# 0411tony/Yue

Measured on AMD Instinct MI355X. Metric: BPR triplet-updates/sec at k=128 (S-round semantics, user rows sequential; the reference's exact sequential semantics: secondary.exact), higher is better.
Workload: dtype f32

## Files before the change

yue_amd/csrc/bpr_host.hip:

```cpp
#include "host_common.hpp"

#include "train_kernels.hpp"
#include "round_kernels.hpp"

using yue_host::fail;
using yue_host::kr_of;
static_assert(yue::kNllSlots == yue_host::kNllSlotsHost && yue::kHeaderSlack == yue_host::kHeaderSlackHost, "host_common.hpp mirrors these");

namespace {

yue::TrainArgs make_args(yue_ctx *c, double lr, double regU, double regI) {
    yue::TrainArgs a{};
    a.P = c->P.p; a.Q = c->Q.p; a.dP = c->dP.p; a.dQ = c->dQ.p;
    a.stage = c->Q.p ? c->Q.p + (size_t)c->n * c->k : nullptr;
    a.ev_u = c->ev_u.p; a.ev_i = c->ev_i.p; a.ev_j = c->ev_j.p;
    a.indptr = c->indptr.p; a.indices = c->indices.p;
    a.nll_slots = c->scal.p;
    a.m = c->m; a.n = c->n; a.k = c->k;
    a.lr = lr;
    a.ru = (float)(lr * regU);
    a.ri = (float)(lr * regI);
    a.neg_lo = 0; a.neg_range = (int32_t)c->n;
    return a;
}
// ... 196 lines not shown
            default: return fail(YUE_ERR_ARG, "item matrices of 2 GiB and more: only the default events-per-wave setting (round_tpw = 0)");
        }
    } else
#define YUE_RM(KR_, TPW_) hipLaunchKernelGGL((yue::k_round_m<KR_, TPW_>), grid, block, 0, c->stream, a, ra, a.ev_u, a.ev_i, a.ev_j, mi, mj); break;
    switch (kr_of(c->k) * 16 + tpw) {
        case 1 * 16 + 8: YUE_RM(1, 8)
        case 1 * 16 + 16: YUE_RM(1, 16)
        case 2 * 16 + 8: YUE_RM(2, 8)
        case 4 * 16 + 4: YUE_RM(4, 4)
        case 1 * 16 + 4: YUE_RM(1, 4)
        case 2 * 16 + 4: YUE_RM(2, 4)
        case 1 * 16 + 2: YUE_RM(1, 2)
        case 2 * 16 + 2: YUE_RM(2, 2)
        default: return fail(YUE_ERR_ARG, "unsupported (k, TPW) combination");
    }
#undef YUE_RM
    launch_round_fold(c, a, e0, e1, round_index);
    return YUE_OK;
}

int launch_round_u(yue_ctx *c, const yue::TrainArgs &a, int64_t u0, int64_t u1, int64_t e0, int64_t e1, int64_t round_index) {
    yue::RoundUArgs ra{};
    ra.u_begin = u0; ra.u_end = u1; ra.ev_ptr = c->d_ev_ptr.p; ra.e_begin = e0; ra.e_end = e1; ra.staged = c->staged ? 1 : 0; ra.margins = c->margins.p;
    const int64_t blocks = (u1 - u0 + 3) / 4;
    if (blocks == 0) return YUE_OK;
    const dim3 grid((unsigned)blocks), block(256);
    const uint32_t *mi = c->meta_i.p, *mj = c->meta_j.p;
#define YUE_RU(KR_) do { if (c->opt_round_fast) hipLaunchKernelGGL((yue::k_round_u<KR_, true>), grid, block, 0, c->stream, a, ra, a.ev_i, a.ev_j, mi, mj); \
                         else hipLaunchKernelGGL((yue::k_round_u<KR_, false>), grid, block, 0, c->stream, a, ra, a.ev_i, a.ev_j, mi, mj); } while (0)
    switch (kr_of(c->k)) {
        case 1: YUE_RU(1); break;
        case 2: YUE_RU(2); break;
        default: YUE_RU(4); break;
    }
#undef YUE_RU
    launch_round_fold(c, a, e0, e1, round_index);
    return YUE_OK;
}

template <typename F>
int run_rounds(yue_ctx *c, yue::TrainArgs a, const std::vector<int64_t> &bounds, int apply_p, F after_round, bool meta = false, const std::vector<int64_t> *user_blocks = nullptr) {
    const int64_t R = (int64_t)bounds.size() - 1;
    int64_t widest = 0;
    for (int64_t r = 0; r < R; ++r) widest = std::max(widest, bounds[(size_t)r + 1] - bounds[(size_t)r]);
    if (widest >= (1ll << 24)) meta = false;
    const bool fits31 = (c->n + 2 * widest) * (int64_t)c->k * 4 < (1ll << 31);
// ... 73 lines not shown
}


}

namespace yue_host {
int zero_scalars(yue_ctx *c) {
    HIPCHK(hipMemsetAsync(c->scal.p, 0, (yue::kNllSlots + 8) * sizeof(double), c->stream));
    return YUE_OK;
}

int read_scalars(yue_ctx *c, double *nll, double *sp, double *sq) {
    double *sc = c->scal.p + yue::kNllSlots;
    hipLaunchKernelGGL(yue::k_sum_slots, dim3(1), dim3(64), 0, c->stream, c->scal.p, yue::kNllSlots, sc);
    double h[3];
    HIPCHK(hipMemcpyAsync(h, sc, sizeof h, hipMemcpyDeviceToHost, c->stream));
    HIPCHK(hipStreamSynchronize(c->stream));
    if (nll) *nll = h[0];
    if (sp) *sp = h[1];
    if (sq) *sq = h[2];
    return YUE_OK;
}

int sumsq_async(yue_ctx *c) {
    double *sc = c->scal.p + yue::kNllSlots;
    HIPCHK(hipMemsetAsync(sc + 1, 0, 2 * sizeof(double), c->stream));
    hipLaunchKernelGGL(yue::k_sumsq, dim3(2048), dim3(256), 0, c->stream, c->P.p, c->m * c->k, sc + 1);
    hipLaunchKernelGGL(yue::k_sumsq, dim3(2048), dim3(256), 0, c->stream, c->Q.p, c->n * c->k, sc + 2);
    return YUE_OK;
}

int upload_triplets(yue_ctx *c, const int32_t *u, const int32_t *i, const int32_t *j, int64_t T, bool validate) {
    for (int64_t t = 0; validate && t < T; ++t) {
        if (u[t] < 0 || u[t] >= c->m || i[t] < 0 || i[t] >= c->n || j[t] >= c->n)
            return fail(YUE_ERR_ARG, "triplet " + std::to_string(t) + " out of range");
    }
    HIPCHK(c->xu.resize((size_t)T + yue::kHeaderSlack)); HIPCHK(c->xi.resize((size_t)T + yue::kHeaderSlack)); HIPCHK(c->xj.resize((size_t)T + yue::kHeaderSlack));
    HIPCHK(hipMemcpyAsync(c->xu.p, u, T * sizeof(int32_t), hipMemcpyHostToDevice, c->stream));
    HIPCHK(hipMemcpyAsync(c->xi.p, i, T * sizeof(int32_t), hipMemcpyHostToDevice, c->stream));
    HIPCHK(hipMemcpyAsync(c->xj.p, j, T * sizeof(int32_t), hipMemcpyHostToDevice, c->stream));
    return YUE_OK;
}
}
using yue_host::zero_scalars; using yue_host::read_scalars; using yue_host::sumsq_async; using yue_host::upload_triplets;

extern "C" {

int yue_bpr_replay(yue_ctx *c, const int32_t *u, const int32_t *i, const int32_t *j, int64_t T,
                   double lr, double regU, double regI, double *nll_out) {
    if (!c || !c->have_factors) return fail(YUE_ERR_ARG, "yue_bpr_replay: no factors uploaded");
// ... 192 lines not shown
    double tot[2] = {(double)E, (double)c->n};
    if (yue_host::on_communicator(c)) {
        if ((rc = yue_allreduce_f64(c, tot, 2))) return rc;
        if ((rc = zero_scalars(c))) return rc;
    }
    const double etot = tot[0];
    if (round_events == 0 && (rc = default_round_events(c, tot[1] / c->nranks, &round_events))) return rc;
    int64_t ub = 1, group = 1;
    if ((rc = yue_epoch_plan(c->m, c->k, round_events, etot, c->nranks, &ub, &group, nullptr))) return rc;
    if (!yue_host::on_communicator(c)) group = std::max<int64_t>(1, (c->m + ub - 1) / ub);
    else group = std::max<int64_t>(1, ((int64_t)c->opt_comm_group_mb << 20) / std::max<int64_t>(1, ub * c->k * 4));
    std::vector<int64_t> ublock;
    for (int64_t u0 = 0; u0 < c->m; u0 += ub) { ublock.push_back(u0); bounds.push_back(c->h_ev_ptr[(size_t)u0]); }
    ublock.push_back(c->m); bounds.push_back(E);
    const int64_t R = (int64_t)ublock.size() - 1;
    const bool seq_user = !yue_host::on_communicator(c) && c->opt_round_user_seq && meta_path_fits(c);
    if (seq_user) {
        HIPCHK(c->d_ev_ptr.resize((size_t)c->m + 1));
        if (!c->d_ev_ptr_valid) {
            HIPCHK(hipMemcpyAsync(c->d_ev_ptr.p, c->h_ev_ptr.data(), ((size_t)c->m + 1) * sizeof(int64_t), hipMemcpyHostToDevice, c->stream));
            c->d_ev_ptr_valid = true;
        }
        HIPCHK(c->margins.resize((size_t)std::max<int64_t>(E, 1)));
    }
    c->last_round_user_seq = 0;
    auto after = [&](int64_t r) -> int {
        if (seq_user && !c->bigq) { c->last_round_user_seq = 1; return YUE_OK; }
        if ((r + 1) % group != 0 && r + 1 != R) return YUE_OK;
        const int64_t g_first = ublock[(size_t)(r - (r % group))], g_last = ublock[(size_t)r + 1];
        const int64_t first = g_first * c->k, count = (g_last - g_first) * c->k;
        const dim3 grid((unsigned)std::min<int64_t>(4096, (count + 255) / 256));
        if (!yue_host::on_communicator(c)) {
            hipLaunchKernelGGL(yue::k_apply_range, grid, dim3(256), 0, c->stream, c->P.p, c->dP.p, first, count);
            return YUE_OK;
        }
        HIPCHK(hipEventRecord(c->ev_rounds, c->stream));
        HIPCHK(hipStreamWaitEvent(c->comm_stream, c->ev_rounds, 0));
        c->comm_collectives += 1;
        c->comm_bytes += (double)count * sizeof(float);
        if (const int rcr = yue_host::reduce_user_block(c, first, count, c->comm_stream)) return rcr;
        hipLaunchKernelGGL(yue::k_apply_range, grid, dim3(256), 0, c->comm_stream, c->P.p, c->dP.p, first, count);
        return YUE_OK;
    };
    c->comm_collectives = 0; c->comm_bytes = 0.0; c->comm_wait_ms = 0.0;
    if ((rc = run_rounds(c, a, bounds, 0, after, meta_path_fits(c), seq_user ? &ublock : nullptr))) { reset_round_state(c); return rc; }
    if (c->last_round_user_seq && E > 0)
        hipLaunchKernelGGL(yue::k_loss_margins, dim3(2048), dim3(256), 0, c->stream, c->margins.p, c->ev_j.p, E, c->scal.p);
    if (yue_host::on_communicator(c)) {
        HIPCHK(hipEventRecord(c->ev_t_rounds, c->stream));
        HIPCHK(hipEventRecord(c->ev_t_comm, c->comm_stream));
    }
    HIPCHK(hipEventRecord(c->ev_comm, c->comm_stream));
    HIPCHK(hipStreamWaitEvent(c->stream, c->ev_comm, 0));
    c->comm_compute_waits = 1;
    HIPCHK(hipGetLastError());
    if ((rc = sumsq_async(c))) return rc;
    if ((rc = read_scalars(c, nll_out, sumsqP_out, sumsqQ_out))) return rc;
    if (yue_host::on_communicator(c)) {
        float ms = 0.f;
        HIPCHK(hipEventSynchronize(c->ev_t_comm));
        HIPCHK(hipEventElapsedTime(&ms, c->ev_t_rounds, c->ev_t_comm));
        c->comm_wait_ms = ms > 0.f ? ms : 0.0;
    }
    return YUE_OK;
}

int yue_epoch_plan(int64_t m, int k, int64_t round_events, double events_total, int nranks,
                   int64_t *user_block, int64_t *blocks_per_group, int64_t *n_blocks) {
    if (m <= 0 || k <= 0 || round_events <= 0 || nranks < 1 || !(events_total >= 0.0)) return fail(YUE_ERR_ARG, "yue_epoch_plan: bad argument");
    const double per_user = events_total / (double)nranks / (double)m;
    const int64_t ub = std::max<int64_t>(1, (int64_t)std::floor((double)round_events / std::max(per_user, 1e-9) + 0.5));
    if (user_block) *user_block = ub;
    if (blocks_per_group) *blocks_per_group = std::max<int64_t>(1, (8ll << 20) / std::max<int64_t>(1, ub * k * 4));
    if (n_blocks) *n_blocks = (m + ub - 1) / ub;
    return YUE_OK;
}

int yue_default_round_events(yue_ctx *c, int64_t *out) {
    if (!c || !c->have_factors || !out) return fail(YUE_ERR_ARG, "yue_default_round_events: upload factors first (the value depends on k)");
// ... 180 lines not shown
```

yue_amd/csrc/core_host.hip:

```cpp
#include "host_common.hpp"

namespace yue_host {
thread_local std::string g_err;
int fail(int code, const std::string &msg) { g_err = msg; return code; }
}
using yue_host::fail;
void yue_comm_release(yue_ctx *c);

extern "C" {

const char *yue_last_error(void) { return yue_host::g_err.c_str(); }
int yue_version(void) { return 1; }

int yue_ctx_create(int device, yue_ctx **out) {
    if (!out) return fail(YUE_ERR_ARG, "yue_ctx_create: out is NULL");
    int ndev = 0;
    HIPCHK(hipGetDeviceCount(&ndev));
    if (ndev <= 0) return fail(YUE_ERR_HIP, "no HIP device visible: libyue_hip needs an MI355X (no CPU fallback exists)");
    if (device < 0 || device >= ndev) return fail(YUE_ERR_ARG, "device ordinal out of range");
    HIPCHK(hipSetDevice(device));
    yue_ctx *c = new yue_ctx();
    c->device = device;
    const auto init = [c]() -> int {
        HIPCHK(hipStreamCreateWithFlags(&c->stream, hipStreamNonBlocking));
// ... 101 lines not shown
    if (indptr[0] != 0 || ev_ptr[0] != 0) return fail(YUE_ERR_ARG, "yue_set_interactions: indptr[0] and ev_ptr[0] must be 0");
    for (int64_t u = 0; u < m; ++u) {
        if (indptr[u + 1] < indptr[u] || ev_ptr[u + 1] < ev_ptr[u]) return fail(YUE_ERR_ARG, "yue_set_interactions: offsets must be non-decreasing");
        for (int64_t t = indptr[u]; t < indptr[u + 1]; ++t) {
            if (indices[t] < 0 || indices[t] >= n) return fail(YUE_ERR_ARG, "yue_set_interactions: item id out of range");
            if (t > indptr[u] && indices[t] <= indices[t - 1]) return fail(YUE_ERR_ARG, "yue_set_interactions: rows must be sorted and unique");
        }
        if (indptr[u + 1] - indptr[u] >= n) return fail(YUE_ERR_ARG, "yue_set_interactions: a user listened to every item (the reference's sampler would never return, BPR.py:47)");
    }
    const int64_t nnz = indptr[m], E = ev_ptr[m];
    {
        int64_t prev = -1, max_gap = 0;
        for (int64_t u = 0; u < m; ++u) if (ev_ptr[u + 1] > ev_ptr[u]) { if (prev >= 0) max_gap = std::max(max_gap, u - prev); prev = u; }
        if (max_gap * c->k * 4 >= (1ll << 31)) return fail(YUE_ERR_ARG, "yue_set_interactions: more than 2 GiB of user-factor rows between two consecutive users with events");
    }
    std::vector<int32_t> evu((size_t)E);
    for (int64_t u = 0; u < m; ++u)
        for (int64_t e = ev_ptr[u]; e < ev_ptr[u + 1]; ++e) {
            if (ev_i[e] < 0 || ev_i[e] >= n) return fail(YUE_ERR_ARG, "yue_set_interactions: event item out of range");
            evu[(size_t)e] = (int32_t)u;
        }
    c->E = E; c->nnz = nnz;
    c->h_ev_ptr.assign(ev_ptr, ev_ptr + m + 1);
    c->d_ev_ptr_valid = false;
    HIPCHK(c->indptr.resize(m + 1)); HIPCHK(c->indices.resize(std::max<int64_t>(nnz, 1)));
    HIPCHK(c->ev_u.resize((size_t)E + yue_host::kHeaderSlackHost)); HIPCHK(c->ev_i.resize((size_t)E + yue_host::kHeaderSlackHost)); HIPCHK(c->ev_j.resize((size_t)E + yue_host::kHeaderSlackHost));
    HIPCHK(hipMemcpyAsync(c->indptr.p, indptr, (m + 1) * sizeof(int64_t), hipMemcpyHostToDevice, c->stream));
    HIPCHK(hipMemcpyAsync(c->indices.p, indices, nnz * sizeof(int32_t), hipMemcpyHostToDevice, c->stream));
    HIPCHK(hipMemcpyAsync(c->ev_u.p, evu.data(), E * sizeof(int32_t), hipMemcpyHostToDevice, c->stream));
    HIPCHK(hipMemcpyAsync(c->ev_i.p, ev_i, E * sizeof(int32_t), hipMemcpyHostToDevice, c->stream));
    HIPCHK(hipStreamSynchronize(c->stream));
    c->have_inter = true;
    return YUE_OK;
}


}
```

yue_amd/csrc/host_common.hpp:

```cpp
#pragma once
#include "../../include/yue_hip.h"

#include <hip/hip_runtime.h>

#include <algorithm>
#include <cmath>
#include <cstdio>
#include <cstdlib>
#include <cstring>
#include <string>
#include <vector>

struct ncclComm;
struct yue_wrmf;
struct yue_knn;
struct yue_ipf;

namespace yue_host {

int fail(int code, const std::string &msg);

#define HIPCHK(expr)                                                                              \
    do {                                                                                          \
        hipError_t e_ = (expr);                                                                   \
// ... 13 lines not shown
        if (e == hipSuccess) n = count;
        return e;
    }
    void release() { if (p) (void)hipFree(p); p = nullptr; n = 0; }
};

constexpr int kNllSlotsHost = 1024;
constexpr int kHeaderSlackHost = 16;

inline int kr_of(int k) { return k <= 64 ? 1 : k <= 128 ? 2 : 4; }

}

using yue_host::DevBuf;

struct yue_ctx {
    int device = 0;
    hipStream_t stream = nullptr;
    int64_t m = 0, n = 0, E = 0, nnz = 0;
    int k = 0;
    bool have_factors = false, have_inter = false;
    DevBuf<float> P, Q, dP, dQ;
    DevBuf<float> margins;
    DevBuf<unsigned long long> cnt0, cnt1;
    DevBuf<uint32_t> cntp0, cntp1;
    DevBuf<uint32_t> tab0, tab1;
    bool staged = false;
    bool bigq = false;
    DevBuf<uint32_t> meta_i, meta_j;
    DevBuf<unsigned long long> round_rows;
    DevBuf<uint2> fold, bk_touch;
    DevBuf<uint32_t> bk_ptr;
    DevBuf<int64_t> d_bounds;
    std::vector<int64_t> h_bounds;
#ifdef YUE_STAMPS
    DevBuf<unsigned long long> stamps;
    int64_t stamp_launch = -1, update_launches = 0, stamp_waves = 0;
#endif
    DevBuf<int32_t> ev_u, ev_i, ev_j, indices;
    DevBuf<int64_t> indptr;
    DevBuf<int32_t> xu, xi, xj, xk;
    DevBuf<double> x_loss;
    DevBuf<float> aU_m, aU_v, aV_m, aV_v;
    int64_t adam_m = 0, adam_n = 0; int adam_k = 0;
    DevBuf<double> scal;
    std::vector<int64_t> h_ev_ptr;
    DevBuf<int32_t> s_users, s_ids, s_mask_idx, s_flags;
    DevBuf<int32_t> s_few, s_few_ids;
    DevBuf<float> s_few_scores;
    int64_t scan_few_users = 0;
    DevBuf<int64_t> s_mask_ptr;
    DevBuf<float> s_scores, s_row, s_norms;
    double scan_ms = 0.0;
    int64_t scan_events = 0, scan_rescored = 0, scan_tiles_done = 0, scan_tiles_total = 0;
    DevBuf<unsigned long long> s_work;
    DevBuf<unsigned short> s_qb;
    DevBuf<uint32_t> s_masks;
    int opt_scan_two_phase = 1;
    int64_t opt_scan_streams_min_users = 262144;
    int opt_scan_slabs = 4;
    int opt_scan_streams = 2;
    int opt_scan_filter_ub = 3;
    int opt_scan_growth = 0;
    int scan_chunks = 0;
    int scan_used_bf16 = 0;
    int opt_scan_f32 = 0;
    int opt_scan_batch = 0;
    int opt_round_tpw = 0;
    int opt_topn_true = 0;
// ... 45 lines not shown
    int64_t chain_runs = 0, chain_waves = 0, chain_groups = 0, chain_kernel_us = 0, replay_levels = 0;
    hipEvent_t ev_chain0 = nullptr, ev_chain1 = nullptr;
    ncclComm *comm = nullptr;
    int rank = 0, nranks = 1;
    hipStream_t comm_stream = nullptr;
    hipEvent_t ev_rounds = nullptr, ev_comm = nullptr;
    hipEvent_t ev_t_rounds = nullptr, ev_t_comm = nullptr;
    int (*seam_reduce)(void *host, int64_t count, int dtype, void *user) = nullptr;
    void *seam_user = nullptr;
    std::vector<float> seam_buf;
    int64_t comm_collectives = 0;
    double comm_bytes = 0.0, comm_wait_ms = 0.0;
    int comm_version = 0, comm_nranks_reported = 0;
    hipEvent_t ev_scan0 = nullptr, ev_scan1 = nullptr;
    yue_wrmf *wrmf = nullptr;
    yue_knn *knn = nullptr;
    yue_ipf *ipf = nullptr;
};

namespace yue_host {
inline bool on_communicator(const yue_ctx *c) { return c->comm != nullptr || c->seam_reduce != nullptr; }
int zero_scalars(yue_ctx *c);
int read_scalars(yue_ctx *c, double *nll, double *sp, double *sq);
int sumsq_async(yue_ctx *c);
int upload_triplets(yue_ctx *c, const int32_t *u, const int32_t *i, const int32_t *j, int64_t T, bool validate);
int reduce_user_block(yue_ctx *c, int64_t first, int64_t count, hipStream_t stream);
int chain_epoch(yue_ctx *c, double lr, double regU, double regI);
int chain_stream(yue_ctx *c, int64_t T, double lr, double regU, double regI);
void wrmf_release(yue_ctx *c);
int wrmf_set_option(yue_ctx *c, const std::string &key, int64_t value);
int wrmf_get_option(yue_ctx *c, const std::string &key, int64_t *value);
void knn_release(yue_ctx *c);
int knn_set_option(yue_ctx *c, const std::string &key, int64_t value);
int knn_get_option(yue_ctx *c, const std::string &key, int64_t *value);
void ipf_release(yue_ctx *c);
int ipf_set_option(yue_ctx *c, const std::string &key, int64_t value);
int ipf_get_option(yue_ctx *c, const std::string &key, int64_t *value);
}
```

yue_amd/csrc/round_kernels.hpp:

```cpp
#pragma once
#include "train_kernels.hpp"

#ifdef YUE_ABL_NO_HOT
#define YUE_M_HOT(val, rs, vo, so) asm volatile("" :: "v"(val))
#else
#define YUE_M_HOT(val, rs, vo, so) YUE_BATOMIC(val, rs, vo, so)
#endif
#ifdef YUE_ABL_NO_DP
#define YUE_M_DP(val, rs, vo, so) asm volatile("" :: "v"(val))
#else
#define YUE_M_DP(val, rs, vo, so) YUE_BATOMIC(val, rs, vo, so)
#endif

#define YUE_BLOAD_NT(rs, vo, so) __builtin_bit_cast(float, __builtin_amdgcn_raw_buffer_load_b32((rs), (vo), (so), 2))
#if defined(YUE_EXP_LOAD_CACHED)
#define YUE_M_LOAD_J(rs, vo, so) YUE_BLOAD(rs, vo, so)
#define YUE_M_LOAD_I(rs, vo, so) YUE_BLOAD(rs, vo, so)
#elif defined(YUE_EXP_LOAD_NT)
#define YUE_M_LOAD_J(rs, vo, so) YUE_BLOAD_NT(rs, vo, so)
#define YUE_M_LOAD_I(rs, vo, so) YUE_BLOAD_NT(rs, vo, so)
#else
#define YUE_M_LOAD_J(rs, vo, so) YUE_BLOAD_NT(rs, vo, so)
#define YUE_M_LOAD_I(rs, vo, so) YUE_BLOAD(rs, vo, so)
#endif

#define YUE_FOLD_LD(p) __builtin_nontemporal_load(p)
#define YUE_FOLD_LDROW(p) (*(p))

namespace yue {

constexpr uint32_t kMetaStageMax = 64u;
constexpr uint32_t kMetaStageDefault = 4u;
constexpr uint32_t kMetaUnique = 1u, kMetaStaged = 2u, kMetaHot = 3u;
constexpr int kMetaUnroll = 8;
__host__ __device__ inline uint32_t meta_kind(uint32_t w) { return w & 3u; }
__host__ __device__ inline uint32_t meta_slot(uint32_t w) { return w >> 2; }
__host__ __device__ inline uint32_t fold_count(uint32_t w) { return w >> 25; }
__host__ __device__ inline uint32_t fold_block(uint32_t w) { return w & 0x1ffffffu; }

struct MetaArgs {
    const int32_t *ev_i, *ev_j;
    const int64_t *bounds;
    int64_t R;
    int32_t n;
    int32_t range;
    int32_t G;
    int32_t chunk;
    uint32_t stage_max;
    uint32_t *meta_i, *meta_j;
    unsigned long long *round_rows;
    uint2 *fold;
    const uint2 *bk_touch;
    const uint32_t *bk_ptr;
};

__host__ __device__ inline int64_t fold_base(int64_t e0, int64_t r) { return (e0 + 4 * r + 3) & ~(int64_t)3; }

template <bool BUCKETED>
__global__ void __launch_bounds__(1024) k_round_meta(MetaArgs a) {
    extern __shared__ uint32_t slots[];
    __shared__ unsigned long long wsum[16];
// ... 42 lines not shown
            const int s = s0 + q;
            if (s < width) { const uint32_t c = slots[s]; if (c >= 2u) mine += (1ull << 32) + (c <= a.stage_max ? c : 0u); }
        }
        unsigned long long incl = mine;
#pragma unroll
        for (int off = 1; off < 64; off <<= 1) { const unsigned long long up = __shfl_up(incl, off); if (lane >= off) incl += up; }
        if (lane == 63) wsum[wv] = incl;
        __syncthreads();
        if (tid == 0) {
            unsigned long long total = 0ull;
            for (int q = 0; q < 16; ++q) total += wsum[q];
            range_base = total ? atomicAdd(a.round_rows + r, total) : 0ull;
        }
        __syncthreads();
        unsigned long long run = range_base + incl - mine;
        for (int q = 0; q < wv; ++q) run += wsum[q];
        uint2 *fold = a.fold + fold_base(e0, r);
        for (int q = 0; q < a.chunk; ++q) {
            const int s = s0 + q;
            if (s < width) {
                const uint32_t c = slots[s];
                if (c >= 2u) {
                    const bool st = c <= a.stage_max;
                    slots[s] = st ? (kMetaStaged | ((uint32_t)run << 2)) : kMetaHot;
                    fold[run >> 32] = make_uint2((uint32_t)(lo + s), st ? ((c << 25) | ((uint32_t)run & 0x1ffffffu)) : 0u);
                    run += (1ull << 32) + (st ? c : 0u);
                }
            }
        }
        __syncthreads();
        if (BUCKETED) {
            for (uint32_t t = tid; t < mine_n; t += 1024) {
                const uint2 tc = mine_t[t];
                const uint32_t sl = tc.x - (uint32_t)lo;
                const uint32_t wd = slots[sl];
                const uint32_t mw = meta_kind(wd) == kMetaStaged ? atomicAdd(&slots[sl], 4u) : wd;
                ((tc.y & 1u) ? a.meta_j : a.meta_i)[e0 + (tc.y >> 1)] = mw;
            }
        } else
        for (int64_t eb = e0 + tid; eb < e1; eb += 1024 * kMetaUnroll) {
            int32_t vi[kMetaUnroll], vj[kMetaUnroll];
#pragma unroll
            for (int q = 0; q < kMetaUnroll; ++q) {
                const int64_t e = eb + 1024 * q;
                vj[q] = e < e1 ? a.ev_j[e] : -1; vi[q] = e < e1 ? a.ev_i[e] : 0;
            }
#pragma unroll
            for (int q = 0; q < kMetaUnroll; ++q) {
                const int64_t e = eb + 1024 * q;
                if (vj[q] >= 0) {
                    const uint32_t si = (uint32_t)(vi[q] - lo), sj = (uint32_t)(vj[q] - lo);
                    if (si < (uint32_t)width) {
                        const uint32_t wd = slots[si];
                        a.meta_i[e] = meta_kind(wd) == kMetaStaged ? atomicAdd(&slots[si], 4u) : wd;
                    }
                    if (sj < (uint32_t)width) {
                        const uint32_t wd = slots[sj];
                        a.meta_j[e] = meta_kind(wd) == kMetaStaged ? atomicAdd(&slots[sj], 4u) : wd;
                    }
                } else if (g == 0 && e < e1) {
                    a.meta_i[e] = 0u; a.meta_j[e] = 0u;
                }
            }
        }
        __syncthreads();
    }
}

constexpr int kBucketShift = 15;
constexpr int kBucketRangesMax = 256;
struct BucketArgs {
    const int32_t *ev_i, *ev_j;
    const int64_t *bounds;
    int64_t R;
    int32_t G;
    uint2 *bk_touch;
    uint32_t *bk_ptr;
    uint32_t *meta_i, *meta_j;
};

__global__ void __launch_bounds__(1024) k_round_bucket(BucketArgs a) {
// ... 139 lines not shown
            const float a1 = p[t][r] * qi[t][r]; ai = ai + a1;
            const float a2 = p[t][r] * qj[t][r]; aj = aj + a2;
        }
        const float x = wave_sum(ai) - wave_sum(aj);
        xs = lane == t ? x : xs;
    }
    __builtin_amdgcn_sched_barrier(0);
    const double s = 1.0 / (1.0 + exp(-(double)xs));
    const float cs = (float)(a.lr * (1.0 - s));
    double nll = (lane < TPW && j >= 0) ? -log(s) : 0.0;
    __builtin_amdgcn_sched_barrier(0);

    YUE_STAMP(3, "");
    float dp[KR];
#pragma unroll
    for (int r = 0; r < KR; ++r) dp[r] = 0.0f;
    bool run_ok = false;
#pragma unroll
    for (int t = 0; t < TPW; ++t) {
        const float c = rdlane(cs, t);
        const unsigned cli = meta_kind(hmi[t]), clj = meta_kind(hmj[t]);
        const bool uniq_i = cli == kMetaUnique, uniq_j = clj == kMetaUnique;
        const bool hot_i = cli == kMetaHot, hot_j = clj == kMetaHot;
        const unsigned wi = uniq_i ? oi[t] : stage0 + meta_slot(hmi[t]) * row_bytes;
        const unsigned wj = uniq_j ? oj[t] : stage0 + meta_slot(hmj[t]) * row_bytes;
        if (ok[t]) {
            run_ok = true;
            Elem o[KR];
#pragma unroll
            for (int r = 0; r < KR; ++r) { o[r] = bpr_elem(p[t][r], qi[t][r], qj[t][r], c, a.ru, a.ri); dp[r] += o[r].p2 - p[t][r]; }
            if (BIGQ) {
                const uint64_t ri_ = (uint64_t)(unsigned)hi_[t] * k, rj_ = (uint64_t)(unsigned)hj[t] * k;
                float *di = hot_i ? a.dQ + ri_ : uniq_i ? a.Q + ri_ : a.stage + (uint64_t)meta_slot(hmi[t]) * k;
                float *dj = hot_j ? a.dQ + rj_ : uniq_j ? a.Q + rj_ : a.stage + (uint64_t)meta_slot(hmj[t]) * k;
#pragma unroll
                for (int r = 0; r < KR; ++r) {
                    if (ev[r]) {
                        if (hot_i) unsafeAtomicAdd(di + el[r], o[r].qi2 - qi[t][r]); else di[el[r]] = uniq_i ? o[r].qi2 : o[r].qi2 - qi[t][r];
                        if (hot_j) unsafeAtomicAdd(dj + el[r], o[r].qj2 - qj[t][r]); else dj[el[r]] = uniq_j ? o[r].qj2 : o[r].qj2 - qj[t][r];
                    }
                }
            } else {
            if (!hot_i) {
#pragma unroll
                for (int r = 0; r < KR; ++r) YUE_BSTORE(uniq_i ? o[r].qi2 : o[r].qi2 - qi[t][r], rsQ, vo[r], wi);
            } else {
#pragma unroll
                for (int r = 0; r < KR; ++r) YUE_M_HOT(o[r].qi2 - qi[t][r], rsdQ, vo[r], oi[t]);
            }
            if (!hot_j) {
#pragma unroll
                for (int r = 0; r < KR; ++r) YUE_BSTORE(uniq_j ? o[r].qj2 : o[r].qj2 - qj[t][r], rsQ, vo[r], wj);
            } else {
#pragma unroll
                for (int r = 0; r < KR; ++r) YUE_M_HOT(o[r].qj2 - qj[t][r], rsdQ, vo[r], oj[t]);
            }
            }
        }
        const bool exists = base + t < ra.e_end;
        const bool last = exists && ((t == TPW - 1) || base + t + 1 >= ra.e_end || ru_[t + 1 < TPW ? t + 1 : t] != ru_[t]);
        if (last) {
            if (run_ok) {
#pragma unroll
                for (int r = 0; r < KR; ++r) YUE_M_DP(dp[r], rsdP, vo[r], ou[t]);
            }
#pragma unroll
            for (int r = 0; r < KR; ++r) dp[r] = 0.0f;
            run_ok = false;
        }
        __builtin_amdgcn_sched_barrier(0);
    }
    YUE_STAMP(4, ""); YUE_STAMP(5, ""); YUE_STAMP(6, "");
#pragma unroll
    for (int off = 1; off < TPW; off <<= 1) nll += __shfl_xor(nll, off);
    if (lane == 0 && nll != 0.0) atomicAdd(a.nll_slots + (wave & (kNllSlots - 1)), nll);
    YUE_STAMP(7, "s_waitcnt vmcnt(0)");
}

struct RoundUArgs {
    int64_t u_begin, u_end;
    const int64_t *ev_ptr;
    int64_t e_begin, e_end;
    int staged;
    float *margins;
};

template <int KR, bool FAST>
__global__ void __launch_bounds__(256) k_round_u(TrainArgs a, RoundUArgs ra, const int32_t *__restrict__ evi, const int32_t *__restrict__ evj,
                                                 const uint32_t *__restrict__ mti, const uint32_t *__restrict__ mtj) {
    const int lane = threadIdx.x & 63;
    const int64_t wave = (int64_t)blockIdx.x * 4 + __builtin_amdgcn_readfirstlane((int)(threadIdx.x >> 6));
    const int64_t u = ra.u_begin + wave;
    if (u >= ra.u_end) return;
    const int64_t e0 = ra.ev_ptr[u], e1 = ra.ev_ptr[u + 1];
    if (e1 <= e0) return;
    const unsigned k = (unsigned)a.k;
    const unsigned row_bytes = k * 4u;
    unsigned vo[KR];
#pragma unroll
    for (int r = 0; r < KR; ++r) { const unsigned e = 64u * r + lane; vo[r] = e < k ? e * 4u : kOobOffset; }
    const uint64_t qbytes = (uint64_t)a.n * row_bytes;
    const int qrec = (int)(qbytes < 0x7fffffffull ? qbytes : 0x7fffffffull);
    const unsigned stage0 = (unsigned)a.n * row_bytes;
    const uint64_t qsbytes = qbytes + (ra.staged ? 2ull * (uint64_t)(ra.e_end - ra.e_begin) * row_bytes : 0ull);
    const int qsrec = (int)(qsbytes < 0x7fffffffull ? qsbytes : 0x7fffffffull);
    const auto rsQ = __builtin_amdgcn_make_buffer_rsrc(a.Q, 0, qsrec, kRsrcFlags);
    const auto rsdQ = __builtin_amdgcn_make_buffer_rsrc(a.dQ, 0, qrec, kRsrcFlags);
// ... 13 lines not shown
            if (!ex) { hI = 0; hJ = -1; hMI = 0u; hMJ = 0u; }
        }
        const unsigned seg_len = len - seg < 64u ? len - seg : 64u;
        float xs = 0.0f;
        auto gather = [&](float (&qi)[KR], float (&qj)[KR], unsigned t) {
            const int ti = __builtin_amdgcn_readlane(hI, t), tj = __builtin_amdgcn_readlane(hJ, t);
            const unsigned oi = (unsigned)ti * row_bytes, oj = (unsigned)(tj < 0 ? 0 : tj) * row_bytes;
#pragma unroll
            for (int r = 0; r < KR; ++r) { qi[r] = YUE_M_LOAD_I(rsQ, vo[r], oi); qj[r] = YUE_M_LOAD_J(rsQ, vo[r], oj); }
        };
        auto step = [&](const float (&qi)[KR], const float (&qj)[KR], unsigned t) {
            const int tj = __builtin_amdgcn_readlane(hJ, t);
            if (tj < 0) return;
            const int ti = __builtin_amdgcn_readlane(hI, t);
            const uint32_t mi = (uint32_t)__builtin_amdgcn_readlane((int)hMI, t), mj = (uint32_t)__builtin_amdgcn_readlane((int)hMJ, t);
            float ai = 0.0f, aj = 0.0f;
#pragma unroll
            for (int r = 0; r < KR; ++r) { const float a1 = p[r] * qi[r]; ai = ai + a1; const float a2 = p[r] * qj[r]; aj = aj + a2; }
            const float x = wave_sum(ai) - wave_sum(aj);
            const float c = FAST ? chain_coef_fast(x, lrf) : (float)(a.lr * (1.0 - chain_sigmoid(x)));
            xs = (unsigned)lane == t ? x : xs;
            const unsigned cli = meta_kind(mi), clj = meta_kind(mj);
            const bool uniq_i = cli == kMetaUnique, uniq_j = clj == kMetaUnique;
            const unsigned oi = (unsigned)ti * row_bytes, oj = (unsigned)tj * row_bytes;
            const unsigned wi = uniq_i ? oi : stage0 + meta_slot(mi) * row_bytes;
            const unsigned wj = uniq_j ? oj : stage0 + meta_slot(mj) * row_bytes;
            Elem o[KR];
#pragma unroll
            for (int r = 0; r < KR; ++r) { o[r] = bpr_elem(p[r], qi[r], qj[r], c, a.ru, a.ri); p[r] = o[r].p2; }
            if (cli != kMetaHot) {
#pragma unroll
                for (int r = 0; r < KR; ++r) YUE_BSTORE(uniq_i ? o[r].qi2 : o[r].qi2 - qi[r], rsQ, vo[r], wi);
            } else {
#pragma unroll
                for (int r = 0; r < KR; ++r) YUE_M_HOT(o[r].qi2 - qi[r], rsdQ, vo[r], oi);
            }
            if (clj != kMetaHot) {
#pragma unroll
                for (int r = 0; r < KR; ++r) YUE_BSTORE(uniq_j ? o[r].qj2 : o[r].qj2 - qj[r], rsQ, vo[r], wj);
            } else {
#pragma unroll
                for (int r = 0; r < KR; ++r) YUE_M_HOT(o[r].qj2 - qj[r], rsdQ, vo[r], oj);
            }
        };
        constexpr int D = KR == 1 ? 8 : 4;
        float qi[D][KR], qj[D][KR];
#pragma unroll
        for (int s_ = 0; s_ < D; ++s_) gather(qi[s_], qj[s_], (unsigned)s_);
        for (unsigned t = 0; t < seg_len; t += D) {
#pragma unroll
            for (int s_ = 0; s_ < D; ++s_) {
                step(qi[s_], qj[s_], t + s_);
                gather(qi[s_], qj[s_], (t + s_ + D) & 63u);
            }
        }
        if ((unsigned)lane < seg_len) ra.margins[e0 + seg + lane] = xs;
    }
#pragma unroll
    for (int r = 0; r < KR; ++r) { const unsigned e = 64u * r + lane; if (e < k) prow[e] = p[r]; }
}

__global__ void __launch_bounds__(256) k_loss_margins(const float *__restrict__ x, const int32_t *__restrict__ evj, int64_t E, double *nll_slots) {
    double nl = 0.0;
    const int64_t stride = (int64_t)gridDim.x * blockDim.x;
    for (int64_t e = (int64_t)blockIdx.x * blockDim.x + threadIdx.x; e < E; e += stride)
        if (evj[e] >= 0) nl += -log(chain_sigmoid(x[e]));
#pragma unroll
    for (int off = 1; off < 64; off <<= 1) nl += __shfl_xor(nl, off);
    if ((threadIdx.x & 63) == 0 && nl != 0.0) atomicAdd(nll_slots + ((blockIdx.x * 4 + (threadIdx.x >> 6)) & (kNllSlots - 1)), nl);
}

struct FoldArgs {
    const uint2 *fold;
    const unsigned long long *round_rows;
    float *Q, *dQ;
    const float *stage;
    int k;
    uint32_t capacity;
};

template <int KR, int EPG>
__device__ __forceinline__ void fold_group(const FoldArgs &f, int lane, unsigned k, uint32_t nact, const uint2 (&ent)[4]) {
    float x[EPG][KR], st[EPG][4][KR];
    unsigned el[KR];
    bool big = false;
#pragma unroll
    for (int r = 0; r < KR; ++r) el[r] = min(64u * r + lane, k - 1u);
#pragma unroll
    for (int sl = 0; sl < EPG; ++sl) {
        if ((uint32_t)sl >= nact) continue;
        const uint32_t c = fold_count(ent[sl].y);
        const bool hot = c == 0u;
        const float *row = f.Q + (uint64_t)ent[sl].x * k;
        const float *src = hot ? f.dQ + (uint64_t)ent[sl].x * k : f.stage + (uint64_t)fold_block(ent[sl].y) * k;
#pragma unroll
        for (int r = 0; r < KR; ++r) { st[sl][0][r] = YUE_FOLD_LD(src + el[r]); if (!hot) st[sl][1][r] = YUE_FOLD_LD(src + (uint64_t)k + el[r]); }
        if (c > 2u) {
#pragma unroll
            for (unsigned q = 2; q < 4; ++q)
#pragma unroll
                for (int r = 0; r < KR; ++r) st[sl][q][r] = YUE_FOLD_LD(src + (uint64_t)(q < c ? q : 0u) * k + el[r]);
        }
        big = big || c > 4u;
#pragma unroll
        for (int r = 0; r < KR; ++r) x[sl][r] = YUE_FOLD_LDROW(row + el[r]);
    }
#pragma unroll
    for (int sl = 0; sl < EPG; ++sl) {
        if ((uint32_t)sl >= nact) continue;
        const uint32_t c = fold_count(ent[sl].y);
        const bool hot = c == 0u;
        float *row = f.Q + (uint64_t)ent[sl].x * k;
        float *dr = f.dQ + (uint64_t)ent[sl].x * k;
#pragma unroll
        for (int r = 0; r < KR; ++r) {
            const unsigned e = 64u * r + lane;
            float acc = st[sl][0][r];
#pragma unroll
            for (unsigned q = 1; q < 4; ++q) { const float v = q < c ? st[sl][q][r] : 0.0f; acc = acc + v; }
            st[sl][0][r] = acc;
            if (c <= 4u && e < k) { row[e] = x[sl][r] + acc; if (hot) dr[e] = 0.0f; }
        }
    }
    if (big) {
#pragma unroll
        for (int sl = 0; sl < EPG; ++sl) {
            if ((uint32_t)sl >= nact) continue;
            const uint32_t c = fold_count(ent[sl].y);
            if (c <= 4u) continue;
            const float *src = f.stage + (uint64_t)fold_block(ent[sl].y) * k;
            float *row = f.Q + (uint64_t)ent[sl].x * k;
            float acc[KR];
#pragma unroll
            for (int r = 0; r < KR; ++r) acc[r] = st[sl][0][r];
            constexpr unsigned STEP = KR == 1 ? 8u : 4u;
            for (uint32_t q0 = 4u; q0 < c; q0 += STEP) {
                float v[STEP][KR];
#pragma unroll
                for (unsigned q = 0; q < STEP; ++q)
#pragma unroll
                    for (int r = 0; r < KR; ++r) v[q][r] = YUE_FOLD_LD(src + (uint64_t)(q0 + q < c ? q0 + q : q0) * k + el[r]);
#pragma unroll
                for (unsigned q = 0; q < STEP; ++q)
#pragma unroll
                    for (int r = 0; r < KR; ++r) acc[r] = acc[r] + (q0 + q < c ? v[q][r] : 0.0f);
            }
#pragma unroll
            for (int r = 0; r < KR; ++r) { const unsigned e = 64u * r + lane; if (e < k) row[e] = x[sl][r] + acc[r]; }
        }
    }
}

template <int KR>
__global__ void __launch_bounds__(256) k_round_fold(FoldArgs f) {
    constexpr int EPG = KR == 4 ? 2 : 4;
    const int lane = threadIdx.x & 63;
    const uint32_t wave = blockIdx.x * 4u + (uint32_t)__builtin_amdgcn_readfirstlane((int)(threadIdx.x >> 6));
    const uint32_t nwaves = gridDim.x * 4u;
    const unsigned k = (unsigned)f.k;
    const uint32_t b0 = wave * EPG;
    uint2 ent[4];
    typedef uint32_t u32x8 __attribute__((ext_vector_type(8)));
    u32x8 ev;
    unsigned long long cntw;
    const bool spec = b0 + 4u <= f.capacity;
    const uint2 *first = f.fold + (spec ? b0 : 0u);
    asm volatile("s_load_dwordx8 %0, %2, 0x0\n\ts_load_dwordx2 %1, %3, 0x0\n\ts_waitcnt lgkmcnt(0)"
                 : "=&s"(ev), "=&s"(cntw) : "s"(first), "s"(f.round_rows) : "memory");
    const uint32_t cnt = (uint32_t)(cntw >> 32);
    ent[0] = make_uint2(ev[0], ev[1]); ent[1] = make_uint2(ev[2], ev[3]); ent[2] = make_uint2(ev[4], ev[5]); ent[3] = make_uint2(ev[6], ev[7]);
    if (b0 < cnt) {
// ... 15 lines not shown
```

Baseline: 1.762 billion.

## Fold P sum-of-squares into round kernel and drop Q reads for staged rows

The per-user round kernel now reduces the squared final P row of each user into slot accumulators, so the separate full k_sumsq pass over P is replaced by a tiny slot sum when every user has events. Staged Q updates change their encoding: the first ticket for an item writes the full new row into its stage slot instead of a delta. The fold kernel then sums the stage slots without reading the old Q row, except for hot rows. This removes one full read of P and one Q row read per staged item, at the cost of extra LDS encoding bits, per-user double atomics, and a different floating-point summation order.

```diff
diff --git a/yue_amd/csrc/bpr_host.hip b/yue_amd/csrc/bpr_host.hip
--- a/yue_amd/csrc/bpr_host.hip
+++ b/yue_amd/csrc/bpr_host.hip
@@ -242,6 +242,7 @@
 int launch_round_u(yue_ctx *c, const yue::TrainArgs &a, int64_t u0, int64_t u1, int64_t e0, int64_t e1, int64_t round_index) {
     yue::RoundUArgs ra{};
     ra.u_begin = u0; ra.u_end = u1; ra.ev_ptr = c->d_ev_ptr.p; ra.e_begin = e0; ra.e_end = e1; ra.staged = c->staged ? 1 : 0; ra.margins = c->margins.p;
+    ra.psq_slots = c->psq_in_rounds ? c->psq_slots.p : nullptr;
     const int64_t blocks = (u1 - u0 + 3) / 4;
     if (blocks == 0) return YUE_OK;
     const dim3 grid((unsigned)blocks), block(256);
@@ -361,10 +362,11 @@
     return YUE_OK;
 }
 
-int sumsq_async(yue_ctx *c) {
+int sumsq_async(yue_ctx *c, const double *p_slots) {
     double *sc = c->scal.p + yue::kNllSlots;
     HIPCHK(hipMemsetAsync(sc + 1, 0, 2 * sizeof(double), c->stream));
-    hipLaunchKernelGGL(yue::k_sumsq, dim3(2048), dim3(256), 0, c->stream, c->P.p, c->m * c->k, sc + 1);
+    if (p_slots) hipLaunchKernelGGL(yue::k_sum_slots, dim3(1), dim3(64), 0, c->stream, p_slots, yue::kNllSlots, sc + 1);
+    else hipLaunchKernelGGL(yue::k_sumsq, dim3(2048), dim3(256), 0, c->stream, c->P.p, c->m * c->k, sc + 1);
     hipLaunchKernelGGL(yue::k_sumsq, dim3(2048), dim3(256), 0, c->stream, c->Q.p, c->n * c->k, sc + 2);
     return YUE_OK;
 }
@@ -603,6 +605,11 @@
             c->d_ev_ptr_valid = true;
         }
         HIPCHK(c->margins.resize((size_t)std::max<int64_t>(E, 1)));
+    }
+    c->psq_in_rounds = seq_user && c->all_users_have_events && E > 0;
+    if (c->psq_in_rounds) {
+        HIPCHK(c->psq_slots.resize((size_t)yue::kNllSlots));
+        HIPCHK(hipMemsetAsync(c->psq_slots.p, 0, (size_t)yue::kNllSlots * sizeof(double), c->stream));
     }
     c->last_round_user_seq = 0;
     auto after = [&](int64_t r) -> int {
@@ -627,6 +634,8 @@
     if ((rc = run_rounds(c, a, bounds, 0, after, meta_path_fits(c), seq_user ? &ublock : nullptr))) { reset_round_state(c); return rc; }
     if (c->last_round_user_seq && E > 0)
         hipLaunchKernelGGL(yue::k_loss_margins, dim3(2048), dim3(256), 0, c->stream, c->margins.p, c->ev_j.p, E, c->scal.p);
+    const bool psq_done = c->psq_in_rounds && c->last_round_user_seq;
+    c->psq_in_rounds = false;
     if (yue_host::on_communicator(c)) {
         HIPCHK(hipEventRecord(c->ev_t_rounds, c->stream));
         HIPCHK(hipEventRecord(c->ev_t_comm, c->comm_stream));
@@ -635,7 +644,7 @@
     HIPCHK(hipStreamWaitEvent(c->stream, c->ev_comm, 0));
     c->comm_compute_waits = 1;
     HIPCHK(hipGetLastError());
-    if ((rc = sumsq_async(c))) return rc;
+    if ((rc = sumsq_async(c, psq_done ? c->psq_slots.p : nullptr))) return rc;
     if ((rc = read_scalars(c, nll_out, sumsqP_out, sumsqQ_out))) return rc;
     if (yue_host::on_communicator(c)) {
         float ms = 0.f;
diff --git a/yue_amd/csrc/core_host.hip b/yue_amd/csrc/core_host.hip
--- a/yue_amd/csrc/core_host.hip
+++ b/yue_amd/csrc/core_host.hip
@@ -147,6 +147,8 @@
         }
     c->E = E; c->nnz = nnz;
     c->h_ev_ptr.assign(ev_ptr, ev_ptr + m + 1);
+    c->all_users_have_events = true;
+    for (int64_t u = 0; u < m; ++u) if (ev_ptr[u + 1] <= ev_ptr[u]) { c->all_users_have_events = false; break; }
     c->d_ev_ptr_valid = false;
     HIPCHK(c->indptr.resize(m + 1)); HIPCHK(c->indices.resize(std::max<int64_t>(nnz, 1)));
     HIPCHK(c->ev_u.resize((size_t)E + yue_host::kHeaderSlackHost)); HIPCHK(c->ev_i.resize((size_t)E + yue_host::kHeaderSlackHost)); HIPCHK(c->ev_j.resize((size_t)E + yue_host::kHeaderSlackHost));
diff --git a/yue_amd/csrc/host_common.hpp b/yue_amd/csrc/host_common.hpp
--- a/yue_amd/csrc/host_common.hpp
+++ b/yue_amd/csrc/host_common.hpp
@@ -59,6 +59,7 @@
     bool have_factors = false, have_inter = false;
     DevBuf<float> P, Q, dP, dQ;
     DevBuf<float> margins;
+    DevBuf<double> psq_slots;
     DevBuf<unsigned long long> cnt0, cnt1;
     DevBuf<uint32_t> cntp0, cntp1;
     DevBuf<uint32_t> tab0, tab1;
@@ -82,6 +83,8 @@
     int64_t adam_m = 0, adam_n = 0; int adam_k = 0;
     DevBuf<double> scal;
     std::vector<int64_t> h_ev_ptr;
+    bool all_users_have_events = false;
+    bool psq_in_rounds = false;
     DevBuf<int32_t> s_users, s_ids, s_mask_idx, s_flags;
     DevBuf<int32_t> s_few, s_few_ids;
     DevBuf<float> s_few_scores;
@@ -173,7 +176,7 @@
 inline bool on_communicator(const yue_ctx *c) { return c->comm != nullptr || c->seam_reduce != nullptr; }
 int zero_scalars(yue_ctx *c);
 int read_scalars(yue_ctx *c, double *nll, double *sp, double *sq);
-int sumsq_async(yue_ctx *c);
+int sumsq_async(yue_ctx *c, const double *p_slots = nullptr);
 int upload_triplets(yue_ctx *c, const int32_t *u, const int32_t *i, const int32_t *j, int64_t T, bool validate);
 int reduce_user_block(yue_ctx *c, int64_t first, int64_t count, hipStream_t stream);
 int chain_epoch(yue_ctx *c, double lr, double regU, double regI);
diff --git a/yue_amd/csrc/round_kernels.hpp b/yue_amd/csrc/round_kernels.hpp
--- a/yue_amd/csrc/round_kernels.hpp
+++ b/yue_amd/csrc/round_kernels.hpp
@@ -32,11 +32,19 @@
 constexpr uint32_t kMetaStageMax = 64u;
 constexpr uint32_t kMetaStageDefault = 4u;
 constexpr uint32_t kMetaUnique = 1u, kMetaStaged = 2u, kMetaHot = 3u;
+constexpr uint32_t kMetaFirst = 1u << 31;
 constexpr int kMetaUnroll = 8;
 __host__ __device__ inline uint32_t meta_kind(uint32_t w) { return w & 3u; }
-__host__ __device__ inline uint32_t meta_slot(uint32_t w) { return w >> 2; }
+__host__ __device__ inline uint32_t meta_slot(uint32_t w) { return (w >> 2) & 0x1fffffffu; }
+__host__ __device__ inline bool meta_first(uint32_t w) { return (w & kMetaFirst) != 0u; }
 __host__ __device__ inline uint32_t fold_count(uint32_t w) { return w >> 25; }
 __host__ __device__ inline uint32_t fold_block(uint32_t w) { return w & 0x1ffffffu; }
+constexpr uint32_t kLdsStaged = 1u << 31, kLdsTicket = 1u << 25;
+static_assert(kMetaStageMax <= 64u, "tickets of a block must fit bits 25..30 of the LDS word");
+__device__ inline uint32_t meta_of_staged(uint32_t lds) {
+    const uint32_t ticket = (lds >> 25) & 63u;
+    return kMetaStaged | (((lds & 0x1ffffffu) + ticket) << 2) | (ticket == 0u ? kMetaFirst : 0u);
+}
 
 struct MetaArgs {
     const int32_t *ev_i, *ev_j;
@@ -125,7 +133,7 @@
                 const uint32_t c = slots[s];
                 if (c >= 2u) {
                     const bool st = c <= a.stage_max;
-                    slots[s] = st ? (kMetaStaged | ((uint32_t)run << 2)) : kMetaHot;
+                    slots[s] = st ? (kLdsStaged | ((uint32_t)run & 0x1ffffffu)) : kMetaHot;
                     fold[run >> 32] = make_uint2((uint32_t)(lo + s), st ? ((c << 25) | ((uint32_t)run & 0x1ffffffu)) : 0u);
                     run += (1ull << 32) + (st ? c : 0u);
                 }
@@ -137,7 +145,7 @@
                 const uint2 tc = mine_t[t];
                 const uint32_t sl = tc.x - (uint32_t)lo;
                 const uint32_t wd = slots[sl];
-                const uint32_t mw = meta_kind(wd) == kMetaStaged ? atomicAdd(&slots[sl], 4u) : wd;
+                const uint32_t mw = (wd & kLdsStaged) ? meta_of_staged(atomicAdd(&slots[sl], kLdsTicket)) : wd;
                 ((tc.y & 1u) ? a.meta_j : a.meta_i)[e0 + (tc.y >> 1)] = mw;
             }
         } else
@@ -155,11 +163,11 @@
                     const uint32_t si = (uint32_t)(vi[q] - lo), sj = (uint32_t)(vj[q] - lo);
                     if (si < (uint32_t)width) {
                         const uint32_t wd = slots[si];
-                        a.meta_i[e] = meta_kind(wd) == kMetaStaged ? atomicAdd(&slots[si], 4u) : wd;
+                        a.meta_i[e] = (wd & kLdsStaged) ? meta_of_staged(atomicAdd(&slots[si], kLdsTicket)) : wd;
                     }
                     if (sj < (uint32_t)width) {
                         const uint32_t wd = slots[sj];
-                        a.meta_j[e] = meta_kind(wd) == kMetaStaged ? atomicAdd(&slots[sj], 4u) : wd;
+                        a.meta_j[e] = (wd & kLdsStaged) ? meta_of_staged(atomicAdd(&slots[sj], kLdsTicket)) : wd;
                     }
                 } else if (g == 0 && e < e1) {
                     a.meta_i[e] = 0u; a.meta_j[e] = 0u;
@@ -345,6 +353,7 @@
         const unsigned cli = meta_kind(hmi[t]), clj = meta_kind(hmj[t]);
         const bool uniq_i = cli == kMetaUnique, uniq_j = clj == kMetaUnique;
         const bool hot_i = cli == kMetaHot, hot_j = clj == kMetaHot;
+        const bool full_i = uniq_i || meta_first(hmi[t]), full_j = uniq_j || meta_first(hmj[t]);
         const unsigned wi = uniq_i ? oi[t] : stage0 + meta_slot(hmi[t]) * row_bytes;
         const unsigned wj = uniq_j ? oj[t] : stage0 + meta_slot(hmj[t]) * row_bytes;
         if (ok[t]) {
@@ -359,21 +368,21 @@
 #pragma unroll
                 for (int r = 0; r < KR; ++r) {
                     if (ev[r]) {
-                        if (hot_i) unsafeAtomicAdd(di + el[r], o[r].qi2 - qi[t][r]); else di[el[r]] = uniq_i ? o[r].qi2 : o[r].qi2 - qi[t][r];
-                        if (hot_j) unsafeAtomicAdd(dj + el[r], o[r].qj2 - qj[t][r]); else dj[el[r]] = uniq_j ? o[r].qj2 : o[r].qj2 - qj[t][r];
+                        if (hot_i) unsafeAtomicAdd(di + el[r], o[r].qi2 - qi[t][r]); else di[el[r]] = full_i ? o[r].qi2 : o[r].qi2 - qi[t][r];
+                        if (hot_j) unsafeAtomicAdd(dj + el[r], o[r].qj2 - qj[t][r]); else dj[el[r]] = full_j ? o[r].qj2 : o[r].qj2 - qj[t][r];
                     }
                 }
             } else {
             if (!hot_i) {
 #pragma unroll
-                for (int r = 0; r < KR; ++r) YUE_BSTORE(uniq_i ? o[r].qi2 : o[r].qi2 - qi[t][r], rsQ, vo[r], wi);
+                for (int r = 0; r < KR; ++r) YUE_BSTORE(full_i ? o[r].qi2 : o[r].qi2 - qi[t][r], rsQ, vo[r], wi);
             } else {
 #pragma unroll
                 for (int r = 0; r < KR; ++r) YUE_M_HOT(o[r].qi2 - qi[t][r], rsdQ, vo[r], oi[t]);
             }
             if (!hot_j) {
 #pragma unroll
-                for (int r = 0; r < KR; ++r) YUE_BSTORE(uniq_j ? o[r].qj2 : o[r].qj2 - qj[t][r], rsQ, vo[r], wj);
+                for (int r = 0; r < KR; ++r) YUE_BSTORE(full_j ? o[r].qj2 : o[r].qj2 - qj[t][r], rsQ, vo[r], wj);
             } else {
 #pragma unroll
                 for (int r = 0; r < KR; ++r) YUE_M_HOT(o[r].qj2 - qj[t][r], rsdQ, vo[r], oj[t]);
@@ -406,6 +415,7 @@
     int64_t e_begin, e_end;
     int staged;
     float *margins;
+    double *psq_slots;
 };
 
 template <int KR, bool FAST>
@@ -465,6 +475,7 @@
             xs = (unsigned)lane == t ? x : xs;
             const unsigned cli = meta_kind(mi), clj = meta_kind(mj);
             const bool uniq_i = cli == kMetaUnique, uniq_j = clj == kMetaUnique;
+            const bool full_i = uniq_i || meta_first(mi), full_j = uniq_j || meta_first(mj);
             const unsigned oi = (unsigned)ti * row_bytes, oj = (unsigned)tj * row_bytes;
             const unsigned wi = uniq_i ? oi : stage0 + meta_slot(mi) * row_bytes;
             const unsigned wj = uniq_j ? oj : stage0 + meta_slot(mj) * row_bytes;
@@ -473,14 +484,14 @@
             for (int r = 0; r < KR; ++r) { o[r] = bpr_elem(p[r], qi[r], qj[r], c, a.ru, a.ri); p[r] = o[r].p2; }
             if (cli != kMetaHot) {
 #pragma unroll
-                for (int r = 0; r < KR; ++r) YUE_BSTORE(uniq_i ? o[r].qi2 : o[r].qi2 - qi[r], rsQ, vo[r], wi);
+                for (int r = 0; r < KR; ++r) YUE_BSTORE(full_i ? o[r].qi2 : o[r].qi2 - qi[r], rsQ, vo[r], wi);
             } else {
 #pragma unroll
                 for (int r = 0; r < KR; ++r) YUE_M_HOT(o[r].qi2 - qi[r], rsdQ, vo[r], oi);
             }
             if (clj != kMetaHot) {
 #pragma unroll
-                for (int r = 0; r < KR; ++r) YUE_BSTORE(uniq_j ? o[r].qj2 : o[r].qj2 - qj[r], rsQ, vo[r], wj);
+                for (int r = 0; r < KR; ++r) YUE_BSTORE(full_j ? o[r].qj2 : o[r].qj2 - qj[r], rsQ, vo[r], wj);
             } else {
 #pragma unroll
                 for (int r = 0; r < KR; ++r) YUE_M_HOT(o[r].qj2 - qj[r], rsdQ, vo[r], oj);
@@ -501,6 +512,14 @@
     }
 #pragma unroll
     for (int r = 0; r < KR; ++r) { const unsigned e = 64u * r + lane; if (e < k) prow[e] = p[r]; }
+    if (ra.psq_slots) {
+        double s = 0.0;
+#pragma unroll
+        for (int r = 0; r < KR; ++r) { const unsigned e = 64u * r + lane; const float sq = p[r] * p[r]; if (e < k) s += (double)sq; }
+#pragma unroll
+        for (int off = 1; off < 64; off <<= 1) s += __shfl_xor(s, off);
+        if (lane == 0) atomicAdd(ra.psq_slots + (u & (kNllSlots - 1)), s);
+    }
 }
 
 __global__ void __launch_bounds__(256) k_loss_margins(const float *__restrict__ x, const int32_t *__restrict__ evj, int64_t E, double *nll_slots) {
@@ -524,7 +543,7 @@
 
 template <int KR, int EPG>
 __device__ __forceinline__ void fold_group(const FoldArgs &f, int lane, unsigned k, uint32_t nact, const uint2 (&ent)[4]) {
-    float x[EPG][KR], st[EPG][4][KR];
+    float st[EPG][4][KR];
     unsigned el[KR];
     bool big = false;
 #pragma unroll
@@ -534,10 +553,17 @@
         if ((uint32_t)sl >= nact) continue;
         const uint32_t c = fold_count(ent[sl].y);
         const bool hot = c == 0u;
-        const float *row = f.Q + (uint64_t)ent[sl].x * k;
         const float *src = hot ? f.dQ + (uint64_t)ent[sl].x * k : f.stage + (uint64_t)fold_block(ent[sl].y) * k;
 #pragma unroll
-        for (int r = 0; r < KR; ++r) { st[sl][0][r] = YUE_FOLD_LD(src + el[r]); if (!hot) st[sl][1][r] = YUE_FOLD_LD(src + (uint64_t)k + el[r]); }
+        for (int r = 0; r < KR; ++r) st[sl][0][r] = YUE_FOLD_LD(src + el[r]);
+        if (hot) {
+            const float *row = f.Q + (uint64_t)ent[sl].x * k;
+#pragma unroll
+            for (int r = 0; r < KR; ++r) st[sl][1][r] = YUE_FOLD_LDROW(row + el[r]);
+        } else {
+#pragma unroll
+            for (int r = 0; r < KR; ++r) st[sl][1][r] = YUE_FOLD_LD(src + (uint64_t)k + el[r]);
+        }
         if (c > 2u) {
 #pragma unroll
             for (unsigned q = 2; q < 4; ++q)
@@ -545,8 +571,6 @@
                 for (int r = 0; r < KR; ++r) st[sl][q][r] = YUE_FOLD_LD(src + (uint64_t)(q < c ? q : 0u) * k + el[r]);
         }
         big = big || c > 4u;
-#pragma unroll
-        for (int r = 0; r < KR; ++r) x[sl][r] = YUE_FOLD_LDROW(row + el[r]);
     }
 #pragma unroll
     for (int sl = 0; sl < EPG; ++sl) {
@@ -558,11 +582,14 @@
 #pragma unroll
         for (int r = 0; r < KR; ++r) {
             const unsigned e = 64u * r + lane;
-            float acc = st[sl][0][r];
-#pragma unroll
-            for (unsigned q = 1; q < 4; ++q) { const float v = q < c ? st[sl][q][r] : 0.0f; acc = acc + v; }
-            st[sl][0][r] = acc;
-            if (c <= 4u && e < k) { row[e] = x[sl][r] + acc; if (hot) dr[e] = 0.0f; }
+            float acc = st[sl][1][r];
+#pragma unroll
+            for (unsigned q = 2; q < 4; ++q) { const float v = q < c ? st[sl][q][r] : 0.0f; acc = acc + v; }
+            st[sl][1][r] = acc;
+            if (c <= 4u && e < k) {
+                row[e] = st[sl][0][r] + acc;
+                if (hot) dr[e] = 0.0f;
+            }
         }
     }
     if (big) {
@@ -575,7 +602,7 @@
             float *row = f.Q + (uint64_t)ent[sl].x * k;
             float acc[KR];
 #pragma unroll
-            for (int r = 0; r < KR; ++r) acc[r] = st[sl][0][r];
+            for (int r = 0; r < KR; ++r) acc[r] = st[sl][1][r];
             constexpr unsigned STEP = KR == 1 ? 8u : 4u;
             for (uint32_t q0 = 4u; q0 < c; q0 += STEP) {
                 float v[STEP][KR];
@@ -589,7 +616,7 @@
                     for (int r = 0; r < KR; ++r) acc[r] = acc[r] + (q0 + q < c ? v[q][r] : 0.0f);
             }
 #pragma unroll
-            for (int r = 0; r < KR; ++r) { const unsigned e = 64u * r + lane; if (e < k) row[e] = x[sl][r] + acc[r]; }
+            for (int r = 0; r < KR; ++r) { const unsigned e = 64u * r + lane; if (e < k) row[e] = st[sl][0][r] + acc[r]; }
         }
     }
 }
```

Result: faster. 1.845 billion (median of 6 runs) (+4.7%).
